# V-Sense/LFBM5D

Hardware: AMD Instinct MI355X
Metric: SAI-megapixels/sec (HT+Wiener, sigma=25) (higher is better)
Workload: dtype f32; 1 GPU; lf17x17x512x512_sigma25; light_field=17x17x512x512x3, asw=1, color_space=opp, noise=MT19937 seed 1 (utilities.cpp:176-183), window_lanes=2, spatial_bands=1, parallelism=single GPU

## Files before the change

### lfbm5d_amd/core.py

```python
import ctypes as C
import os
import subprocess

from typing import NamedTuple, Optional

import numpy as np

_HERE = os.path.dirname(os.path.abspath(__file__))

YUV, YCBCR, OPP, RGB, ID, DCT, SADCT, BIOR, HADAMARD, HAAR = range(10)
ROWMAJOR, COLMAJOR = 11, 12
TAU = {"id": ID, "dct": DCT, "sadct": SADCT, "bior": BIOR, "hw": HADAMARD, "haar": HAAR}
COLOR_SPACE = {"yuv": YUV, "ycbcr": YCBCR, "opp": OPP, "rgb": RGB}
UNIQUE_ID_BYTES = 128
SR_BICUBIC, SR_GAUSSIAN = 0, 1
SR_UP, SR_DOWN = 0, 1
SR_KERNEL = {"bicubic": SR_BICUBIC, "gaussian": SR_GAUSSIAN}


class LfBm5dError(RuntimeError):
    pass


class Params(C.Structure):
# ... 274 lines not shown
    out = (C.c_void_p * len(arrays))()
    for i, a in enumerate(arrays):
        if a is None or not mask[i]:
            continue
        if not (isinstance(a, np.ndarray) and a.dtype == np.float32 and a.flags.c_contiguous):
            raise LfBm5dError("per-SAI host buffers must be contiguous float32 numpy arrays")
        out[i] = a.ctypes.data
    return out


OPTION_ENV = ("LFBM5D_LANES", "LFBM5D_EMULATE_WORLD", "LFBM5D_MAX_WINDOWS", "LFBM5D_FUSED", "LFBM5D_STEP_SHARDING",
              "LFBM5D_DATA_DRIVEN_SCHEDULE", "LFBM5D_HOST_BLOCKING", "LFBM5D_BAND_MB", "LFBM5D_BM3D_LANES", "LFBM5D_SCAN_LDS_CAP",
              "LFBM5D_FORCE_REDO", "LFBM5D_SPATIAL_BANDS", "LFBM5D_BAND_HALO", "LFBM5D_SCAN_V1", "LFBM5D_SCAN_ANY", "LFBM5D_SCAN_FULL_TABLES", "LFBM5D_DCT8W_V2",
              "LFBM5D_GROUP_GENERIC", "LFBM5D_NO_SA_KERNELS", "LFBM5D_NO_SLAB_KERNEL", "LFBM5D_WIDE_NOSPLIT", "LFBM5D_AGG_64BIT",
              "LFBM5D_AGG_SCALAR_SCAN", "LFBM5D_SUBSET_LIST_HOST", "LFBM5D_SUBSET_SCAN_V1", "LFBM5D_FILT_GROUP_MAJOR",
              "LFBM5D_HT_REF_ORDER", "LFBM5D_WINDOW_SUMS_PADDED")
OPTION_ENV_EMPTY_OFF = ("LFBM5D_WINDOW_SUMS_PADDED",)


class Context:

    def __init__(self, device=0):
        self._L = lib()
        h = C.c_void_p()
        if self._L.lfbm5d_create(C.byref(h), int(device)) != 0:
            raise LfBm5dError(self._L.lfbm5d_last_error(None).decode())
        self._handle = h
        self._env_seen = {k: os.environ.get(k) for k in OPTION_ENV}
        self.device = int(device)

    @property
# ... 330 lines not shown
```

### lfbm5d_amd/csrc/lfbm5d_aggregate.hip

```cpp
#include "lfbm5d_kernels.h"

#include <algorithm>
#include <cstdlib>

namespace lfbm5d {

namespace {



constexpr int kAggFlush = 64;
template <bool WINDOWED, int TW, int TH, int kAggPF, int kAggU, bool BIG, bool VEC4>
__global__ __launch_bounds__(64) __attribute__((amdgpu_waves_per_eu((VEC4 && TW == 8 && !BIG) ? 8 : 1))) void k_aggregate(AggArgs a) {
    constexpr int kAggCap = kAggFlush + kAggPF * 64 + kAggU;
    __shared__ uint4 hit_a[kAggCap];
    __shared__ float hit_w2[kAggCap];
    __shared__ float kai[WINDOWED ? 256 : 1];
    const int lane = threadIdx.x;
    const unsigned org = a.direct ? a.nHW : 0u, Wt = a.Wb - 2 * org, Ht = a.Hb - 2 * org;
    const unsigned gx = (Wt + TW - 1) / TW, gy = (Ht + TH - 1) / TH, total_wg = gx * gy * a.A;
    const unsigned per_xcd = gridDim.x / 8;
    const unsigned lin2 = (blockIdx.x % 8) * per_xcd + blockIdx.x / 8;
    if (lin2 >= total_wg) return;
    const int st = (int)(lin2 / (gx * gy));
    const int tile_y = (int)((lin2 / gx) % gy), tile_x = (int)(lin2 % gx);
    if (a.proc_bits.test((unsigned)st)) return;
    if (!a.mask_bits.test((unsigned)st)) return;
    const int tx0 = (int)org + tile_x * TW, ty0 = (int)org + tile_y * TH;
    const int x = tx0 + lane % TW, y = ty0 + lane / TW;
    const bool inside = x < (int)(org + Wt) && y < (int)(org + Ht);
    const int k = a.k, k2 = k * k, C = a.C, N = a.N, A = a.A;
// ... 26 lines not shown
    const size_t pix = (a.direct ? (size_t)a.sai.st[st] * a.lf_stride : (size_t)st * C * plane) + (size_t)(y - (int)org) * Wt + (size_t)(x - (int)org);
    if (inside) for (int c = 0; c < C; c++) { accn[c] = a.num[pix + c * plane]; accd[c] = a.den[pix + c * plane]; }

    const bool mul_div = !a.irregular && (long long)n_rr * ncols_span < (1 << 20);
    const unsigned div_m = ((1u << 20) + (unsigned)max(ncols_span, 1) - 1) / (unsigned)max(ncols_span, 1);
    const unsigned g_end = a.ref_begin + a.n_groups;
    const bool sai_major = a.filt_sai_stride != 0;
    const unsigned Af = sai_major ? 1u : (unsigned)A, stf = sai_major ? 0u : (unsigned)st;
    const float* const filt = a.filt + (sai_major ? (size_t)st * a.filt_sai_stride : (size_t)0);
    const unsigned long long filt_bytes = sai_major ? a.filt_sai_stride * sizeof(float) : a.filt_bytes;
    const bool small24 = (((unsigned long long)a.n_refs_total << logN) + 1) * Af < (1ull << 24);
    const unsigned* apos = a.aggpos + (size_t)st * a.n_refs_total * N;
    const unsigned cstride = C > 1 ? (unsigned)k2 * 4u : 0u;
    const __amdgpu_buffer_rsrc_t rs_filt = __builtin_amdgcn_make_buffer_rsrc((void*)filt, 0, BIG ? 0 : (int)(unsigned)filt_bytes, 0x00020000u);
    unsigned nh = 0;

    auto consume = [&]() {
        const unsigned nh_pad = (nh + kAggU - 1) / kAggU * kAggU;
        if (nh + lane < nh_pad) { hit_a[nh + lane] = make_uint4(0xffffffffu, 0u, 0u, 0u); hit_w2[nh + lane] = 0.0f; }
        __builtin_amdgcn_wave_barrier();
        for (unsigned h0 = 0; h0 < nh_pad; h0 += kAggU) {
            float val[kAggU][3], kw[kAggU][3];
#pragma unroll
            for (int u = 0; u < kAggU; u++) {
                const uint4 ha = hit_a[h0 + u];
                const float w2 = hit_w2[h0 + u];
                const int dy = y - (int)(ha.x >> 16), dx = x - (int)(ha.x & 0xffffu);
                const bool on = (unsigned)dy < (unsigned)k && (unsigned)dx < (unsigned)k;
                const unsigned o = __umul24((unsigned)min(max(dy, 0), k - 1), (unsigned)k) + (unsigned)min(max(dx, 0), k - 1);
                const float kz = WINDOWED ? kai[o] : 1.0f;
                if (BIG) {
                    const char* fp = reinterpret_cast<const char*>(filt) + ((size_t)ha.y + o) * 4;
                    val[u][0] = *reinterpret_cast<const float*>(fp);
                    val[u][1] = *reinterpret_cast<const float*>(fp + cstride);
                    val[u][2] = *reinterpret_cast<const float*>(fp + 2 * cstride);
                } else {
                    const int vo = (int)((ha.y + o) * 4u);
                    val[u][0] = __builtin_bit_cast(float, __builtin_amdgcn_raw_buffer_load_b32(rs_filt, vo, 0, kFiltLoadAux));
                    val[u][1] = __builtin_bit_cast(float, __builtin_amdgcn_raw_buffer_load_b32(rs_filt, vo, (int)cstride, kFiltLoadAux));
                    val[u][2] = __builtin_bit_cast(float, __builtin_amdgcn_raw_buffer_load_b32(rs_filt, vo, (int)(2 * cstride), kFiltLoadAux));
                }
                kw[u][0] = on ? kz * __uint_as_float(ha.z) : 0.0f;
                kw[u][1] = on ? kz * __uint_as_float(ha.w) : 0.0f;
                kw[u][2] = on ? kz * w2 : 0.0f;
            }
// ... 43 lines not shown
            auto below = [&](unsigned long long b) { return __builtin_amdgcn_mbcnt_hi((unsigned)(b >> 32), __builtin_amdgcn_mbcnt_lo((unsigned)b, 0u)); };
            const unsigned total = (unsigned)__popcll(b0) + 2u * (unsigned)__popcll(b1) + 4u * (unsigned)__popcll(b2);
            if (nh + total > cap_hits) return false;
            if (m4) {
                unsigned slot = nh + below(b0) + 2u * below(b1) + 4u * below(b2);
                size_t wbase; unsigned off;
                const unsigned gl = g - a.ref_begin;
                if (small24) { wbase = __umul24(g, (unsigned)C); off = __umul24(__umul24((gl << logN) + n0, Af) + stf, (unsigned)(C * k2)); }
                else { asm volatile("" ::: "memory"); wbase = (size_t)g * C; off = (((gl << logN) + n0) * Af + stf) * C * k2; }
                float w[3];
#pragma unroll
                for (int c = 0; c < 3; c++) w[c] = c < C ? a.wgt[wbase + (a.wchan0 ? 0 : c)] : 0.0f;
#pragma unroll
                for (int j = 0; j < 4; j++) {
                    if (m4 & (1u << j)) {
                        hit_a[slot] = make_uint4(pj[j], off, __float_as_uint(w[0]), __float_as_uint(w[1]));
                        hit_w2[slot] = w[2];
                        slot++;
                    }
                    off += pstep;
                }
            }
            nh += total;
            __builtin_amdgcn_wave_barrier();
            return true;
        };
        for (int c0 = 0; c0 < n_cand; c0 += 256) {
            if (!try_append(c0, 0u, 64u))
                for (unsigned l0 = 0; l0 < 64; l0 += 16) { consume(); (void)try_append(c0, l0, l0 + 16); }
            if (nh >= kAggFlush) consume();
        }
    } else
// ... 30 lines not shown
        for (int u = 0; u < kAggPF; u++) {
            const int py = (int)(p[u] >> 16), px = (int)(p[u] & 0xffffu);
            hit[u] = p[u] != 0xffffffffu && py < ty0 + TH && py + k > ty0 && px < tx0 + TW && px + k > tx0;
#pragma unroll
            for (int c = 0; c < 3; c++) w[u][c] = (hit[u] && c < C) ? a.wgt[wbase[u] + (a.wchan0 ? 0 : c)] : 0.0f;
        }
#pragma unroll
        for (int u = 0; u < kAggPF; u++) {
            const unsigned long long bal = __ballot(hit[u]);
            if (hit[u]) {
                const unsigned slot = nh + __popcll(bal & ((1ull << lane) - 1ull));
                unsigned off;
                const unsigned gl = g[u] - a.ref_begin;
                if (small24) off = __umul24(__umul24((gl << logN) + nn[u], Af) + stf, (unsigned)(C * k2));
                else { asm volatile("" ::: "memory"); off = (((gl << logN) + nn[u]) * Af + stf) * C * k2; }
                hit_a[slot] = make_uint4(p[u], off, __float_as_uint(w[u][0]), __float_as_uint(w[u][1]));
                hit_w2[slot] = w[u][2];
            }
            nh += __popcll(bal);
        }
        __builtin_amdgcn_wave_barrier();
        if (nh >= kAggFlush) consume();
    }
    if (nh) consume();
    if (inside) for (int c = 0; c < C; c++) { a.num[pix + c * plane] = accn[c]; a.den[pix + c * plane] = accd[c]; }
}

}

hipError_t launch_aggregate(hipStream_t s, const AggArgs& a) {
    const bool wide = a.k >= 12;
    constexpr int kAgg16TW = 16, kAgg16TH = 4, kAgg8TW = 8, kAgg8TH = 8;
    const unsigned tw = wide ? (a.k == 12 ? 16 : kAgg16TW) : (a.k == 8 ? kAgg8TW : 8), th = wide ? (a.k == 12 ? 4 : kAgg16TH) : (a.k == 8 ? kAgg8TH : 8);
    const unsigned org = a.direct ? a.nHW : 0u;
    const unsigned tiles = ((a.Wb - 2 * org + tw - 1) / tw) * ((a.Hb - 2 * org + th - 1) / th) * a.A;
    const dim3 grid(((tiles + 7) / 8) * 8), block(64);
    const bool big = (a.filt_sai_stride ? a.filt_sai_stride * sizeof(float) : a.filt_bytes) > 0xfffff000ull || (a.opt & kOptAgg64Bit);
    const bool vec4 = a.N % 4 == 0 && !wide && !(a.opt & kOptAggScalarScan);
#define LFBM5D_AGG(W_, TW_, TH_, PF_, U_) \
    do { if (big && vec4) hipLaunchKernelGGL((k_aggregate<W_, TW_, TH_, PF_, U_, true, true>), grid, block, 0, s, a); \
         else if (big)    hipLaunchKernelGGL((k_aggregate<W_, TW_, TH_, PF_, U_, true, false>), grid, block, 0, s, a); \
         else if (vec4)   hipLaunchKernelGGL((k_aggregate<W_, TW_, TH_, PF_, U_, false, true>), grid, block, 0, s, a); \
         else             hipLaunchKernelGGL((k_aggregate<W_, TW_, TH_, PF_, U_, false, false>), grid, block, 0, s, a); } while (0)
    constexpr int kAgg16PF = 3, kAgg16U = 12, kAgg8PF = 3, kAgg8U = 6;
    if (a.k == 12)      LFBM5D_AGG(true, 16, 4, 3, 12);
    else if (a.k == 8)  LFBM5D_AGG(true, kAgg8TW, kAgg8TH, kAgg8PF, kAgg8U);
    else if (wide)      LFBM5D_AGG(false, kAgg16TW, kAgg16TH, kAgg16PF, kAgg16U);
    else                LFBM5D_AGG(false, 8, 8, 2, 6);
#undef LFBM5D_AGG
    return hipGetLastError();
}

}
```

### lfbm5d_amd/csrc/lfbm5d_group_generic.hip

```cpp
#include "lfbm5d_group_device.h"

namespace lfbm5d {

namespace {

__global__ __launch_bounds__(256) void k_group_pos(GroupArgs a) {
    const int A = a.A, N = a.N, NA = N * A;
    const size_t plane = (size_t)a.Wb * a.Hb;
    const size_t idx = (size_t)blockIdx.x * blockDim.x + threadIdx.x;
    if (idx == 0 && a.sa_list) a.sa_list[0] = 0u;
    if (idx >= (size_t)a.n_groups * N) return;
    const unsigned g = a.ref_begin + (unsigned)(idx / N);
    const int n = (int)(idx % N);
    const int nSx = (int)a.self_cnt[g];
    const unsigned k_r = a.refs[g];
    const unsigned ind_pst = n < nSx ? a.self_idx[(size_t)g * N + n] : 0u;
    const bool want_ofs = A == 9 && a.tau2 == 4 && a.step == 1 && (size_t)A * a.C * plane * 4 < 0x7fffffffull;
    unsigned bits = 0;
    for (int st = 0; st < A; st++) {
        const bool masked = a.mask_bits.test((unsigned)st);
        unsigned p = 0xffffffffu;
        if (n < nSx && masked) p = (st == (int)a.pst) ? ind_pst : a.best[(size_t)st * plane + ind_pst];
        const bool zero_patch = a.fill_quirk && p != 0xffffffffu && (p % a.Wb) >= a.Wb - a.k;
        const int i = n * A + st;
        a.gpos[(size_t)g * NA + i] = zero_patch ? 0xffffffffu : p;
        if (want_ofs) {
            const bool there = !zero_patch && p != 0xffffffffu;
            a.gofs[(size_t)g * NA + i] = there ? (unsigned)(((size_t)st * a.C * plane + p) * 4) : 0u;
            bits |= there ? 1u << st : 0u;
        }
        const bool in_shape = st == (int)a.pst || (masked && a.shape[(size_t)st * plane + k_r]);
        a.aggpos[((size_t)st * a.n_refs_total + g) * N + n] = ((a.tau4 != 6 || in_shape) && p != 0xffffffffu) ? ((p / a.Wb) << 16) | (p % a.Wb) : 0xffffffffu;
    }
    if (want_ofs) a.gok[(size_t)g * N + n] = bits;
}
template <bool BIG>
__global__ __launch_bounds__(256) void k_group_shape(GroupArgs a) {
    typedef typename std::conditional<BIG, ShapeInfoBig, ShapeInfo>::type SH;
    const unsigned i = blockIdx.x * blockDim.x + threadIdx.x;
    if (i >= a.n_groups) return;
    const unsigned g = a.ref_begin + i;
    const size_t plane = (size_t)a.Wb * a.Hb;
    const unsigned k_r = a.refs[g];
    SH* out = reinterpret_cast<SH*>(a.gshape) + g;
    if (a.tau4 != 6) { out->use_sadct = 0; return; }
    const int A = (int)a.A, aw = window_side(A);
    if (BIG) {
        int* m = out->mask_dct;
        int full = 0;
// ... 318 lines not shown
```

### lfbm5d_amd/csrc/lfbm5d_group_ht.hip

```cpp
#include "lfbm5d_group_device.h"

namespace lfbm5d {

namespace {

__device__ __forceinline__ constexpr float ht_guard(int st) { return st == 0 ? 1.0f / 65536.0f : (st == 3 || st == 6) ? 1.0f / 131072.0f : 1.0f / 262144.0f; }
template <int NS> __device__ __forceinline__ void haar_fwd_pairs_u(v2f* P) {
    if (NS == 8) {
        const v2f S01 = P[0] + P[1], D01 = P[0] - P[1], S23 = P[2] + P[3], D23 = P[2] - P[3];
        const v2f SS = S01 + S23, DD = S01 - S23;
        P[0] = v2f{SS.x + SS.y, SS.x - SS.y}; P[1] = DD; P[2] = D01; P[3] = D23;
    } else if (NS == 4) {
        const v2f S = P[0] + P[1], D = P[0] - P[1];
        P[0] = v2f{S.x + S.y, S.x - S.y}; P[1] = D;
    } else if (NS == 2) {
        P[0] = v2f{P[0].x + P[0].y, P[0].x - P[0].y};
    }
}
template <int NS> __device__ __forceinline__ void haar_inv_pairs_u(v2f* P) {
    if (NS == 8) {
        const v2f X = v2f{P[0].x + P[0].y, P[0].x - P[0].y};
        const v2f U = P[1] * 2.0f + X, V = X - P[1] * 2.0f, D01 = P[2], D23 = P[3];
        P[0] = D01 * 4.0f + U; P[1] = U - D01 * 4.0f; P[2] = D23 * 4.0f + V; P[3] = V - D23 * 4.0f;
    } else if (NS == 4) {
// ... 163 lines not shown
}

template <int NS, bool HAAR, bool LDSW = false, int SA_MODE = 0, bool FAST = false>
__device__ __forceinline__ bool group_id_body(const GroupArgs& a, unsigned g, int c, int pq, const __attribute__((address_space(4))) unsigned* pos,
                                              ShRef sh, bool use_sadct, float& wacc, float& s1, float& s2, float* work = nullptr) {
    const int k = a.k, k2 = k * k, A = 9;
    const unsigned plane = a.Wb * a.Hb;
    const unsigned kRsrcFlags = 0x00020000u;
    const __amdgpu_buffer_rsrc_t rs_in = __builtin_amdgcn_make_buffer_rsrc((void*)a.noisy, 0, (int)((size_t)a.A * a.C * plane * 4), kRsrcFlags);
    float* const out = a.filt + (size_t)g * a.N * A * a.C * k2;
    const __amdgpu_buffer_rsrc_t rs_out = __builtin_amdgcn_make_buffer_rsrc((void*)out, 0, (int)((size_t)a.N * A * a.C * k2 * 4), kRsrcFlags);
    constexpr int NH = NS > 1 ? NS / 2 : 1;
    v2f V[NH][9];
    const int voff = (int)(((unsigned)(pq / k) * a.Wb + pq % k) * 4u);
    const int woff = (pq / k) * (k + 1) + pq % k;
    unsigned okbits[NS];
    typedef const __attribute__((address_space(4))) unsigned* cuptr_;
    const cuptr_ ofs = (cuptr_)(a.gofs + (size_t)g * a.N * A), ok = (cuptr_)(a.gok + (size_t)g * a.N);
    const unsigned cbase = (unsigned)c * plane * 4u;
    auto load_all = [&]() {
        if (LDSW) {
#pragma unroll
            for (int n = 0; n < NS; n++)
#pragma unroll
                for (int st = 0; st < 9; st++) {
                    const float x = work[(n * A + st) * kT16Patch + woff];
                    if (n < NH) V[n][st].x = x; else V[n - NH][st].y = x;
                    okbits[n] = 0x1ffu;
                }
        } else
#pragma unroll
        for (int n = 0; n < NS; n++) {
            okbits[n] = ok[n];
#pragma unroll
            for (int st = 0; st < 9; st++) {
                const unsigned so = ofs[n * A + st] + cbase;
                const float x = __builtin_bit_cast(float, __builtin_amdgcn_raw_buffer_load_b32(rs_in, voff, (int)so, 0));
                if (n < NH) V[n][st].x = x; else V[n - NH][st].y = x;
            }
        }
        if (NS == 1) {
#pragma unroll
            for (int st = 0; st < 9; st++) V[0][st].y = 0.0f;
        }
#pragma unroll
        for (int n = 0; n < NS; n++)
            if (okbits[n] != 0x1ffu) {
#pragma unroll
                for (int st = 0; st < 9; st++) {
                    if (n < NH) V[n][st].x = ((okbits[n] >> st) & 1) ? V[n][st].x : 0.0f;
                    else V[n - NH][st].y = ((okbits[n] >> st) & 1) ? V[n - NH][st].y : 0.0f;
                }
            }
    };
    load_all();
    bool near = false;
    if (FAST) near = group_id_compute_fast<NS>(a, c, V, wacc, s1, s2);
    else
    group_id_compute<NS, HAAR, SA_MODE>(a, c, sh, use_sadct, V, wacc, s1, s2);
    const int vout = pq * 4;
#pragma unroll
    for (int n = 0; n < NS; n++)
#pragma unroll
        for (int st = 0; st < 9; st++) {
            const float r = n < NH ? V[n][st].x : V[n - NH][st].y;
            if (LDSW) work[(n * A + st) * kT16Patch + woff] = r;
            else __builtin_amdgcn_raw_buffer_store_b32(__builtin_bit_cast(int, r), rs_out, vout, (int)((((unsigned)(n * A + st) * a.C + c) * k2) * 4u), kFiltStoreAux);
        }
    return near;
}

template <bool HAAR, int SA_MODE, bool FAST = false>
__device__ __forceinline__ void group_id_one(const GroupArgs& a, const unsigned g, const int c, float (*red)[4]) {
    const int tid = threadIdx.x;
    const int A = 9, N = a.N;
    const int nSx = (int)a.self_cnt[g];
    typedef const __attribute__((address_space(4))) unsigned* cuptr;
    const cuptr pos = (cuptr)(a.gpos + (size_t)g * N * A);
    ShRef sh = group_shape(a, g);
    const bool use_sadct = a.tau4 == 6 && sh.use_sadct;
    if (SA_MODE == 3 && use_sadct) return;
    float wacc = 0.0f, s1 = 0.0f, s2 = 0.0f;
// ... 311 lines not shown
}

hipError_t prepare_group_ht() {
    const void* fns[] = {
        reinterpret_cast<const void*>(&k_group_bior16_haar), reinterpret_cast<const void*>(&k_group_bior16_any),
        reinterpret_cast<const void*>(&k_group_dct16_haar), reinterpret_cast<const void*>(&k_group_dct16_any),
        reinterpret_cast<const void*>(&k_group_bior16_n1), reinterpret_cast<const void*>(&k_group_dct16_n1),
        reinterpret_cast<const void*>(&k_group_bior16_n1_sa), reinterpret_cast<const void*>(&k_group_dct16_n1_sa)};
    for (const void* f : fns) {
        const hipError_t e = hipFuncSetAttribute(f, hipFuncAttributeMaxDynamicSharedMemorySize, kDedicatedLdsLimit);
        if (e != hipSuccess) return e;
    }
    return hipSuccess;
}

hipError_t launch_group_ht(hipStream_t s, const GroupArgs& a, bool all_sa, bool* launched) {
    *launched = true;
    if (a.tau2 == 4 && a.N <= 8 && a.k * a.k <= 256 && a.step == 1 && a.A == 9 && (size_t)a.A * a.C * a.Wb * a.Hb * 4 < 0x7fffffffull) {
        const unsigned threads = ((a.k * a.k + 63) / 64) * 64;
        const unsigned gx = ((a.n_groups + 7) / 8) * 8;
        if (all_sa) {
            if (a.tau5 == 9) hipLaunchKernelGGL(k_group_id_haar_sa, dim3(gx, a.C), dim3(threads), 0, s, a);
            else             hipLaunchKernelGGL(k_group_id_any_sa, dim3(gx, a.C), dim3(threads), 0, s, a);
        }
        else {
            if (!a.sa_list) return hipErrorInvalidValue;
            const bool fast = a.tau5 == 9 && (a.tau4 == 5 || a.tau4 == 6) && a.C <= 3 && !(a.opt & kOptHtReferenceOrder);
            if (fast)             hipLaunchKernelGGL(k_group_id_haar_fast, dim3(gx, a.C), dim3(threads), 0, s, a);
            else if (a.tau5 == 9) hipLaunchKernelGGL(k_group_id_haar, dim3(gx, a.C), dim3(threads), 0, s, a);
            else                  hipLaunchKernelGGL(k_group_id_any, dim3(gx, a.C), dim3(threads), 0, s, a);
            if (a.tau4 == 6 || fast) {
                if (a.tau5 == 9) hipLaunchKernelGGL(k_group_id_haar_list, dim3(kSaListBlocks), dim3(threads), 0, s, a);
                else             hipLaunchKernelGGL(k_group_id_any_list, dim3(kSaListBlocks), dim3(threads), 0, s, a);
// ... 32 lines not shown
```

### lfbm5d_amd/csrc/lfbm5d_kernels.h

```cpp
#ifndef LFBM5D_KERNELS_H
#define LFBM5D_KERNELS_H

#include <hip/hip_runtime.h>
#include <vector>

#include "lfbm5d_options.h"

constexpr int kFiltStoreAux = 2;
constexpr int kFiltLoadAux = 0;

#if defined(__HIPCC__)
typedef float filt_v4f __attribute__((ext_vector_type(4)));
typedef float filt_v2f __attribute__((ext_vector_type(2)));
__device__ __forceinline__ void filt_put(float* p, const float v) { *p = v; }
__device__ __forceinline__ void filt_put2(filt_v2f* p, const filt_v2f v) { *p = v; }
__device__ __forceinline__ void filt_put4(filt_v4f* p, const filt_v4f v) { *p = v; }
__device__ __forceinline__ void filt_put4(float4* p, const float4 v) { *p = v; }
__device__ __forceinline__ void filt_put4_nt(filt_v4f* p, const filt_v4f v) { __builtin_nontemporal_store(v, p); }
#endif

namespace lfbm5d {

constexpr int kMaxK = 32;
constexpr int kMaxA = 49;
// ... 69 lines not shown
    unsigned ref_begin, n_groups;
    unsigned Wb, Hb, C, A, k, N, pst;
    SaiMask mask_bits, proc_bits;
    unsigned tau2, tau4, tau5, useSD;
    unsigned fill_quirk;
    int step;
    float lambda;
    float sigma[3];
    float ht3_T[3][9][4];
    float ht3_K[3][9];
    float* scratch;
    unsigned long long scratch_floats;
    unsigned opt;
    unsigned long long filt_sai_stride;
    unsigned bm3d;
};

constexpr unsigned kSaiMajorMinA = 121;
__device__ __forceinline__ size_t filt_patch(const GroupArgs& a, unsigned g, unsigned n, unsigned st, unsigned k2) {
    return a.filt_sai_stride ? (size_t)st * a.filt_sai_stride + ((size_t)g * a.N + n) * a.C * k2
                             : (((size_t)g * a.N + n) * a.A + st) * a.C * k2;
}


struct SaiList { unsigned st[kBigA]; unsigned n; };

struct AggArgs {
    float* num;
    float* den;
    const float* filt;
// ... 6 lines not shown
    const unsigned* self_idx;
    const unsigned* self_cnt;
    const unsigned* best;
    const unsigned char* shape;
    const GroupTables* tb;
    unsigned ref_begin, n_groups;
    unsigned n_ref_rows, n_ref_cols;
    unsigned Wb, Hb, C, A, k, N, pst, p, nHW, nSim, nDisp;
    SaiMask mask_bits, proc_bits; unsigned tau4;
    unsigned irregular;
    unsigned opt;
    unsigned wchan0;
    unsigned direct;
    unsigned long long lf_stride;
    SaiList sai;
};

__host__ __device__ inline size_t stereo_table_stride(unsigned W, unsigned H, unsigned k, unsigned nDisp) {
    const unsigned ncols = W - 2 * nDisp - (k - 1), nrows = H - 2 * nDisp - (k - 1);
    return (size_t)((ncols + 63) / 64) * 64 * (nrows + 63);
}

__host__ __device__ inline unsigned stereo_table_srq(unsigned H, unsigned k, unsigned nDisp) {
    const unsigned nrows = H - 2 * nDisp - (k - 1);
    return ((nrows - 1 + 63 + 15) / 16) * 4 + 1;
}
__host__ __device__ inline size_t stereo_table_stride2(unsigned W, unsigned H, unsigned k, unsigned nDisp) {
    const unsigned ncols = W - 2 * nDisp - (k - 1);
    return (size_t)((ncols - 1 + 63) / 64) * stereo_table_srq(H, k, nDisp) * 256 + stereo_table_srq(H, k, nDisp) * 4;
}
// ... 106 lines not shown
                                 unsigned* best, unsigned char* shape);
hipError_t launch_stereo_argmin2(hipStream_t s, const float* tables, const unsigned* st_of_slot, unsigned n_slots,
                                 unsigned W, unsigned H, unsigned k, unsigned nDisp, float thr,
                                 unsigned* best, unsigned char* shape);
hipError_t launch_self_select(hipStream_t s, const float* scores, const unsigned* refs, unsigned n_refs,
                              unsigned W, unsigned nSim, unsigned N, float thr, unsigned* self_idx,
                              unsigned* self_cnt,
                              unsigned grid_cols = 0, unsigned nHW = 0, unsigned p = 1, unsigned last_r = 0, unsigned last_c = 0);
hipError_t launch_self_trivial(hipStream_t s, const unsigned* refs, unsigned n_refs, unsigned* self_idx,
                               unsigned* self_cnt);
hipError_t launch_stereo_argmin(hipStream_t s, const float* tables, const unsigned* st_of_slot, unsigned n_slots,
                                unsigned W, unsigned H, unsigned k, unsigned nDisp, float thr,
                                unsigned* best, unsigned char* shape);
hipError_t prepare_group_kernels();
hipError_t launch_group(hipStream_t s, const GroupArgs& a);
size_t group_lds_bytes(const GroupArgs& a);
size_t group_scratch_bytes(const GroupArgs& a);
hipError_t launch_aggregate(hipStream_t s, const AggArgs& a);

}
#endif
```

### lfbm5d_amd/csrc/lfbm5d_options.h

```cpp
#ifndef LFBM5D_OPTIONS_H
#define LFBM5D_OPTIONS_H

#include <cstddef>
#include <cstdlib>
#include <cstring>
#include <string>

namespace lfbm5d {

enum : unsigned {
    kOptScanV1 = 1u << 0,
    kOptScanAny = 1u << 1,
    kOptScanFullTables = 1u << 2,
    kOptDct8wV2 = 1u << 3,
    kOptGroupGeneric = 1u << 4,
    kOptNoSaKernels = 1u << 5,
    kOptNoSlabKernel = 1u << 6,
    kOptWideNoSplit = 1u << 7,
    kOptAgg64Bit = 1u << 8,
    kOptAggScalarScan = 1u << 9,
    kOptSubsetListHost = 1u << 10,
    kOptSubsetScanV1 = 1u << 11,
    kOptFiltGroupMajor = 1u << 12,
    kOptHtReferenceOrder = 1u << 13,
};

struct Options {
    int lanes = 2;
    int emulate_world = 0;
    int max_windows = 0;
    int fused = 1;
    int step_sharding = 0;
    int data_driven_schedule = 0;
    int host_blocking = 0;
    int band_mb = 0;
    int bm3d_lanes = 3;
    int scan_lds_cap = 0;
    int force_redo = 0;
    int spatial_bands = 1;
// ... 11 lines not shown
        {"step_sharding", "LFBM5D_STEP_SHARDING", &Options::step_sharding, 0},
        {"data_driven_schedule", "LFBM5D_DATA_DRIVEN_SCHEDULE", &Options::data_driven_schedule, 0},
        {"host_blocking", "LFBM5D_HOST_BLOCKING", &Options::host_blocking, 0}, {"band_mb", "LFBM5D_BAND_MB", &Options::band_mb, 0},
        {"bm3d_lanes", "LFBM5D_BM3D_LANES", &Options::bm3d_lanes, 0}, {"scan_lds_cap", "LFBM5D_SCAN_LDS_CAP", &Options::scan_lds_cap, 0},
        {"force_redo", "LFBM5D_FORCE_REDO", &Options::force_redo, 0}, {"spatial_bands", "LFBM5D_SPATIAL_BANDS", &Options::spatial_bands, 0},
        {"band_halo", "LFBM5D_BAND_HALO", &Options::band_halo, 0},
        {"window_sums_padded", "LFBM5D_WINDOW_SUMS_PADDED", &Options::window_sums_padded, 0},
        {"scan_v1", "LFBM5D_SCAN_V1", nullptr, kOptScanV1}, {"scan_any", "LFBM5D_SCAN_ANY", nullptr, kOptScanAny},
        {"scan_full_tables", "LFBM5D_SCAN_FULL_TABLES", nullptr, kOptScanFullTables}, {"dct8w_v2", "LFBM5D_DCT8W_V2", nullptr, kOptDct8wV2},
        {"group_generic", "LFBM5D_GROUP_GENERIC", nullptr, kOptGroupGeneric}, {"no_sa_kernels", "LFBM5D_NO_SA_KERNELS", nullptr, kOptNoSaKernels},
        {"no_slab_kernel", "LFBM5D_NO_SLAB_KERNEL", nullptr, kOptNoSlabKernel}, {"wide_nosplit", "LFBM5D_WIDE_NOSPLIT", nullptr, kOptWideNoSplit},
        {"agg_64bit", "LFBM5D_AGG_64BIT", nullptr, kOptAgg64Bit}, {"agg_scalar_scan", "LFBM5D_AGG_SCALAR_SCAN", nullptr, kOptAggScalarScan},
        {"subset_list_host", "LFBM5D_SUBSET_LIST_HOST", nullptr, kOptSubsetListHost}, {"subset_scan_v1", "LFBM5D_SUBSET_SCAN_V1", nullptr, kOptSubsetScanV1},
        {"filt_group_major", "LFBM5D_FILT_GROUP_MAJOR", nullptr, kOptFiltGroupMajor},
        {"ht_reference_order", "LFBM5D_HT_REF_ORDER", nullptr, kOptHtReferenceOrder},
    };
    *n = sizeof(keys) / sizeof(keys[0]);
    return keys;
}

inline bool option_set(Options& o, const char* key, const char* value) {
    size_t n; const OptionKey* keys = option_keys(&n);
    static const Options defaults;
    for (size_t i = 0; i < n; i++) {
        if (std::strcmp(key, keys[i].key) != 0 && std::strcmp(key, keys[i].env) != 0) continue;
        const bool unset = value == nullptr || value[0] == 0;
        if (keys[i].field) {
            int v = defaults.*(keys[i].field);
            if (!unset) {
                if (keys[i].field == &Options::step_sharding) v = std::strcmp(value, "rows") == 0 ? 1 : std::strcmp(value, "blocks") == 0 ? 2 : std::atoi(value);
// ... 36 lines not shown
```

### lfbm5d_amd/csrc/lfbm5d_pass.hip

```cpp
#include "lfbm5d_ctx.h"

namespace lfbm5d_host {

lfbm5d_ctx* new_ctx(int device, std::string& err) {
    hipError_t e;
    lfbm5d_ctx* c = new lfbm5d_ctx();
    c->device = device;
    std::memset(&c->stats, 0, sizeof(c->stats));
    if ((e = hipStreamCreateWithFlags(&c->stream, hipStreamNonBlocking)) != hipSuccess) { err = hipGetErrorString(e); delete c; return nullptr; }
    if ((e = prepare_group_kernels()) != hipSuccess || (e = prepare_scan2_kernels()) != hipSuccess) { err = std::string("kernel LDS limits: ") + hipGetErrorString(e); (void)hipStreamDestroy(c->stream); delete c; return nullptr; }
    if ((e = hipHostMalloc((void**)&c->h_small, 64 * sizeof(unsigned))) != hipSuccess) { err = hipGetErrorString(e); (void)hipStreamDestroy(c->stream); delete c; return nullptr; }
    return c;
}


hipEvent_t get_event(lfbm5d_ctx* c) {
    if (c->ev_used == c->ev_pool.size()) {
        hipEvent_t e; (void)hipEventCreate(&e); c->ev_pool.push_back(e);
    }
    return c->ev_pool[c->ev_used++];
}

void drain_events(lfbm5d_ctx* c) {
    for (const PassEvents& pe : c->pending) {
// ... 260 lines not shown
    {
        constexpr size_t kFiltCapBytes = (size_t)12 << 30;
        size_t cap = std::min<size_t>(kFiltCapBytes, (size_t)0xfff00000ull * sizeof(float));
        if (c->opt->band_mb > 0) cap = std::min<size_t>(cap, (size_t)c->opt->band_mb << 20);
        const size_t row_groups = centre ? gc.n_ref_cols : 1;
        if ((size_t)R * per_group * sizeof(float) > cap) {
            const size_t rows_fit = std::max<size_t>(1, cap / (per_group * sizeof(float) * row_groups));
            band_groups = (unsigned)std::min<size_t>(R, rows_fit * row_groups);
        }
    }
    HIPCK(c, c->filt.reserve((size_t)band_groups * per_group * sizeof(float)));
    HIPCK(c, c->wgt.reserve((size_t)R * C * sizeof(float)));
    HIPCK(c, c->aggpos.reserve((size_t)A * R * Nst * sizeof(unsigned)));
    HIPCK(c, c->gpos.reserve((size_t)A * R * Nst * sizeof(unsigned)));
    HIPCK(c, c->gofs.reserve((size_t)A * R * Nst * sizeof(unsigned)));
    HIPCK(c, c->gok.reserve((size_t)R * Nst * sizeof(unsigned)));
    HIPCK(c, c->sa_list.reserve((size_t)(4 * (size_t)R + 1) * sizeof(unsigned)));
    HIPCK(c, c->gshape.reserve((size_t)R * (A > (unsigned)kMaxA ? kShapeInfoBigBytes : kShapeInfoBytes)));
    HIPCK(c, gc.tb.reserve(sizeof(GroupTables)));
    if (!c->counters.p) {
        HIPCK(c, c->counters.reserve(32 * sizeof(unsigned long long)));
        HIPCK(c, hipMemsetAsync(c->counters.p, 0, 32 * sizeof(unsigned long long), s));
    }
    unsigned long long* const d_counters = c->counters.as<unsigned long long>() + 16 * c->gslot;
    if (gc.tb_key[0] != k || gc.tb_key[1] != aw || gc.tb_key[2] != ah) {
        GroupTables tb;
        build_tables(tb, k, aw, ah);
        HIPCK(c, hipMemcpyAsync(gc.tb.p, &tb, sizeof(tb), hipMemcpyHostToDevice, s));
        HIPCK(c, hipStreamSynchronize(s));
        gc.tb_key[0] = k; gc.tb_key[1] = aw; gc.tb_key[2] = ah;
    }
// ... 109 lines not shown
    ga.opt = c->opt->kernels;
    if (const size_t sb = group_scratch_bytes(ga)) {
        HIPCK(c, c->gscratch.reserve(sb));
        ga.scratch = c->gscratch.as<float>(); ga.scratch_floats = sb / sizeof(float);
    }
    AggArgs aa;
    std::memset(&aa, 0, sizeof(aa));
    aa.num = d_num; aa.den = d_den; aa.wgt = ga.wgt; aa.aggpos = ga.aggpos; aa.n_refs_total = R; aa.refs = ga.refs;
    aa.self_idx = ga.self_idx; aa.self_cnt = ga.self_cnt; aa.best = ga.best; aa.shape = ga.shape; aa.tb = ga.tb;
    aa.ref_begin = ref_begin; aa.n_groups = n_groups; aa.n_ref_rows = gc.n_ref_rows; aa.n_ref_cols = gc.n_ref_cols;
    aa.Wb = Wb; aa.Hb = Hb; aa.C = C; aa.A = A; aa.k = k; aa.N = Nst; aa.pst = pst; aa.p = P->p;
    aa.nHW = nHW; aa.nSim = P->nSim; aa.nDisp = P->nDisp;
    aa.mask_bits = mask_bits; aa.proc_bits = proc_bits; aa.tau4 = P->tau_4D; aa.irregular = centre ? 0u : 1u;
    aa.wchan0 = (bm3d && P->useSD) ? 1u : 0u;
    aa.opt = c->opt->kernels;
    if (direct) {
        aa.num = c->direct.num; aa.den = c->direct.den; aa.direct = 1u; aa.lf_stride = c->direct.lf_stride; aa.sai = c->direct.sai;
    }
    const bool sai_major = A >= kSaiMajorMinA && !(c->opt->kernels & kOptFiltGroupMajor);
    const size_t per_group_bias = sai_major ? per_group / A : per_group;
    if (n_groups <= band_groups) {
        ga.filt_sai_stride = aa.filt_sai_stride = sai_major ? (unsigned long long)n_groups * (per_group / A) : 0ull;
        ga.filt = c->filt.as<float>() - (size_t)ref_begin * per_group_bias;
        aa.filt = c->filt.as<float>(); aa.filt_bytes = (unsigned long long)n_groups * per_group * sizeof(float);
        if (n_groups) HIPCK(c, launch_group(s, ga));
        HIPCK(c, hipEventRecord(pe.e[2], s));
        if (n_groups) HIPCK(c, launch_aggregate(s, aa));
        HIPCK(c, hipEventRecord(pe.e[3], s));
    } else {
        bool first = true;
// ... 57 lines not shown
```

Baseline: 252.9 SAI-megapixels/s.

## Store filtered HT patches in tile-split row-block layout for aggregation locality

Adds a split layout for filtered group patches when k=16. The HT group kernel writes each patch split at the aggregation tile boundary into left and right pieces. Within each piece, rows are blocked in groups of 4, so an aggregation tile reads its columns from contiguous memory. The group kernel stores a per-SAI split column in an extra gok word, and the aggregate kernel gets a BR template instance that recomputes offsets from the piece width. This trades more offset arithmetic, extra LDS and a doubled gok buffer for better-coalesced filter loads in aggregation. It is on by default and can be turned off with LFBM5D_FILT_ROWS.

Measured after the change: 250.2 SAI-megapixels/s. -1.0%, worse.

```diff
diff --git a/lfbm5d_amd/core.py b/lfbm5d_amd/core.py
--- a/lfbm5d_amd/core.py
+++ b/lfbm5d_amd/core.py
@@ -312,7 +312,7 @@
               "LFBM5D_FORCE_REDO", "LFBM5D_SPATIAL_BANDS", "LFBM5D_BAND_HALO", "LFBM5D_SCAN_V1", "LFBM5D_SCAN_ANY", "LFBM5D_SCAN_FULL_TABLES", "LFBM5D_DCT8W_V2",
               "LFBM5D_GROUP_GENERIC", "LFBM5D_NO_SA_KERNELS", "LFBM5D_NO_SLAB_KERNEL", "LFBM5D_WIDE_NOSPLIT", "LFBM5D_AGG_64BIT",
               "LFBM5D_AGG_SCALAR_SCAN", "LFBM5D_SUBSET_LIST_HOST", "LFBM5D_SUBSET_SCAN_V1", "LFBM5D_FILT_GROUP_MAJOR",
-              "LFBM5D_HT_REF_ORDER", "LFBM5D_WINDOW_SUMS_PADDED")
+              "LFBM5D_HT_REF_ORDER", "LFBM5D_WINDOW_SUMS_PADDED", "LFBM5D_FILT_ROWS")
 OPTION_ENV_EMPTY_OFF = ("LFBM5D_WINDOW_SUMS_PADDED",)
 
 
diff --git a/lfbm5d_amd/csrc/lfbm5d_aggregate.hip b/lfbm5d_amd/csrc/lfbm5d_aggregate.hip
--- a/lfbm5d_amd/csrc/lfbm5d_aggregate.hip
+++ b/lfbm5d_amd/csrc/lfbm5d_aggregate.hip
@@ -10,11 +10,12 @@
 
 
 constexpr int kAggFlush = 64;
-template <bool WINDOWED, int TW, int TH, int kAggPF, int kAggU, bool BIG, bool VEC4>
+template <bool WINDOWED, int TW, int TH, int kAggPF, int kAggU, bool BIG, bool VEC4, int BR>
 __global__ __launch_bounds__(64) __attribute__((amdgpu_waves_per_eu((VEC4 && TW == 8 && !BIG) ? 8 : 1))) void k_aggregate(AggArgs a) {
     constexpr int kAggCap = kAggFlush + kAggPF * 64 + kAggU;
     __shared__ uint4 hit_a[kAggCap];
     __shared__ float hit_w2[kAggCap];
+    __shared__ unsigned short hit_pw[BR ? kAggCap : 1];
     __shared__ float kai[WINDOWED ? 256 : 1];
     const int lane = threadIdx.x;
     const unsigned org = a.direct ? a.nHW : 0u, Wt = a.Wb - 2 * org, Ht = a.Hb - 2 * org;
@@ -71,10 +72,19 @@
     const unsigned cstride = C > 1 ? (unsigned)k2 * 4u : 0u;
     const __amdgpu_buffer_rsrc_t rs_filt = __builtin_amdgcn_make_buffer_rsrc((void*)filt, 0, BIG ? 0 : (int)(unsigned)filt_bytes, 0x00020000u);
     unsigned nh = 0;
+    auto piece_bias = [&](const unsigned pos) -> unsigned {
+        if (!BR) return 0u;
+        const int px = (int)(pos & 0xffffu);
+        return filt_piece_bias(TW, BR, filt_split_s(TW, px, (int)org), px >= tx0);
+    };
+    auto piece_w = [&](const unsigned pos) -> unsigned {
+        const int px = (int)(pos & 0xffffu);
+        return filt_piece_w(TW, filt_split_s(TW, px, (int)org), px >= tx0);
+    };
 
     auto consume = [&]() {
         const unsigned nh_pad = (nh + kAggU - 1) / kAggU * kAggU;
-        if (nh + lane < nh_pad) { hit_a[nh + lane] = make_uint4(0xffffffffu, 0u, 0u, 0u); hit_w2[nh + lane] = 0.0f; }
+        if (nh + lane < nh_pad) { hit_a[nh + lane] = make_uint4(0xffffffffu, 0u, 0u, 0u); hit_w2[nh + lane] = 0.0f; if (BR) hit_pw[nh + lane] = (unsigned short)TW; }
         __builtin_amdgcn_wave_barrier();
         for (unsigned h0 = 0; h0 < nh_pad; h0 += kAggU) {
             float val[kAggU][3], kw[kAggU][3];
@@ -84,8 +94,9 @@
                 const float w2 = hit_w2[h0 + u];
                 const int dy = y - (int)(ha.x >> 16), dx = x - (int)(ha.x & 0xffffu);
                 const bool on = (unsigned)dy < (unsigned)k && (unsigned)dx < (unsigned)k;
-                const unsigned o = __umul24((unsigned)min(max(dy, 0), k - 1), (unsigned)k) + (unsigned)min(max(dx, 0), k - 1);
-                const float kz = WINDOWED ? kai[o] : 1.0f;
+                const unsigned orow = __umul24((unsigned)min(max(dy, 0), k - 1), (unsigned)k) + (unsigned)min(max(dx, 0), k - 1);
+                const float kz = WINDOWED ? kai[orow] : 1.0f;
+                const unsigned o = BR ? filt_piece_offset(TW, BR, (unsigned)hit_pw[BR ? h0 + u : 0], min(max(dy, 0), TW - 1), min(max(dx, 0), TW - 1)) : orow;
                 if (BIG) {
                     const char* fp = reinterpret_cast<const char*>(filt) + ((size_t)ha.y + o) * 4;
                     val[u][0] = *reinterpret_cast<const float*>(fp);
@@ -159,8 +170,9 @@
 #pragma unroll
                 for (int j = 0; j < 4; j++) {
                     if (m4 & (1u << j)) {
-                        hit_a[slot] = make_uint4(pj[j], off, __float_as_uint(w[0]), __float_as_uint(w[1]));
+                        hit_a[slot] = make_uint4(pj[j], off + piece_bias(pj[j]), __float_as_uint(w[0]), __float_as_uint(w[1]));
                         hit_w2[slot] = w[2];
+                        if (BR) hit_pw[slot] = (unsigned short)piece_w(pj[j]);
                         slot++;
                     }
                     off += pstep;
@@ -221,8 +233,9 @@
                 const unsigned gl = g[u] - a.ref_begin;
                 if (small24) off = __umul24(__umul24((gl << logN) + nn[u], Af) + stf, (unsigned)(C * k2));
                 else { asm volatile("" ::: "memory"); off = (((gl << logN) + nn[u]) * Af + stf) * C * k2; }
-                hit_a[slot] = make_uint4(p[u], off, __float_as_uint(w[u][0]), __float_as_uint(w[u][1]));
+                hit_a[slot] = make_uint4(p[u], off + piece_bias(p[u]), __float_as_uint(w[u][0]), __float_as_uint(w[u][1]));
                 hit_w2[slot] = w[u][2];
+                if (BR) hit_pw[slot] = (unsigned short)piece_w(p[u]);
             }
             nh += __popcll(bal);
         }
@@ -237,23 +250,26 @@
 
 hipError_t launch_aggregate(hipStream_t s, const AggArgs& a) {
     const bool wide = a.k >= 12;
-    constexpr int kAgg16TW = 16, kAgg16TH = 4, kAgg8TW = 8, kAgg8TH = 8;
-    const unsigned tw = wide ? (a.k == 12 ? 16 : kAgg16TW) : (a.k == 8 ? kAgg8TW : 8), th = wide ? (a.k == 12 ? 4 : kAgg16TH) : (a.k == 8 ? kAgg8TH : 8);
+    constexpr int kAgg16TW = agg_tile(16).tw, kAgg16TH = agg_tile(16).th, kAgg16BR = agg_tile(16).br, kAgg8TW = agg_tile(8).tw, kAgg8TH = agg_tile(8).th;
+    static_assert(agg_tile(12).tw == 16 && agg_tile(12).th == 4 && agg_tile(6).tw == 8 && agg_tile(6).th == 8 && kAgg16BR > 0 && kAgg16TW == 16, "instances below");
+    const unsigned tw = (unsigned)agg_tile(a.k).tw, th = (unsigned)agg_tile(a.k).th;
+    if (a.filt_split && !(a.k == 16 && agg_tile(a.k).br)) return hipErrorInvalidValue;
     const unsigned org = a.direct ? a.nHW : 0u;
     const unsigned tiles = ((a.Wb - 2 * org + tw - 1) / tw) * ((a.Hb - 2 * org + th - 1) / th) * a.A;
     const dim3 grid(((tiles + 7) / 8) * 8), block(64);
     const bool big = (a.filt_sai_stride ? a.filt_sai_stride * sizeof(float) : a.filt_bytes) > 0xfffff000ull || (a.opt & kOptAgg64Bit);
     const bool vec4 = a.N % 4 == 0 && !wide && !(a.opt & kOptAggScalarScan);
-#define LFBM5D_AGG(W_, TW_, TH_, PF_, U_) \
-    do { if (big && vec4) hipLaunchKernelGGL((k_aggregate<W_, TW_, TH_, PF_, U_, true, true>), grid, block, 0, s, a); \
-         else if (big)    hipLaunchKernelGGL((k_aggregate<W_, TW_, TH_, PF_, U_, true, false>), grid, block, 0, s, a); \
-         else if (vec4)   hipLaunchKernelGGL((k_aggregate<W_, TW_, TH_, PF_, U_, false, true>), grid, block, 0, s, a); \
-         else             hipLaunchKernelGGL((k_aggregate<W_, TW_, TH_, PF_, U_, false, false>), grid, block, 0, s, a); } while (0)
+#define LFBM5D_AGG(W_, TW_, TH_, PF_, U_, BR_) \
+    do { if (big && vec4) hipLaunchKernelGGL((k_aggregate<W_, TW_, TH_, PF_, U_, true, true, BR_>), grid, block, 0, s, a); \
+         else if (big)    hipLaunchKernelGGL((k_aggregate<W_, TW_, TH_, PF_, U_, true, false, BR_>), grid, block, 0, s, a); \
+         else if (vec4)   hipLaunchKernelGGL((k_aggregate<W_, TW_, TH_, PF_, U_, false, true, BR_>), grid, block, 0, s, a); \
+         else             hipLaunchKernelGGL((k_aggregate<W_, TW_, TH_, PF_, U_, false, false, BR_>), grid, block, 0, s, a); } while (0)
     constexpr int kAgg16PF = 3, kAgg16U = 12, kAgg8PF = 3, kAgg8U = 6;
-    if (a.k == 12)      LFBM5D_AGG(true, 16, 4, 3, 12);
-    else if (a.k == 8)  LFBM5D_AGG(true, kAgg8TW, kAgg8TH, kAgg8PF, kAgg8U);
-    else if (wide)      LFBM5D_AGG(false, kAgg16TW, kAgg16TH, kAgg16PF, kAgg16U);
-    else                LFBM5D_AGG(false, 8, 8, 2, 6);
+    if (a.k == 12)      LFBM5D_AGG(true, 16, 4, 3, 12, 0);
+    else if (a.k == 8)  LFBM5D_AGG(true, kAgg8TW, kAgg8TH, kAgg8PF, kAgg8U, 0);
+    else if (a.filt_split) LFBM5D_AGG(false, kAgg16TW, kAgg16TH, kAgg16PF, kAgg16U, kAgg16BR);
+    else if (wide)      LFBM5D_AGG(false, kAgg16TW, kAgg16TH, kAgg16PF, kAgg16U, 0);
+    else                LFBM5D_AGG(false, 8, 8, 2, 6, 0);
 #undef LFBM5D_AGG
     return hipGetLastError();
 }
diff --git a/lfbm5d_amd/csrc/lfbm5d_filt_layout.h b/lfbm5d_amd/csrc/lfbm5d_filt_layout.h
--- /dev/null
+++ b/lfbm5d_amd/csrc/lfbm5d_filt_layout.h
@@ -0,0 +1,43 @@
+#ifndef LFBM5D_FILT_LAYOUT_H
+#define LFBM5D_FILT_LAYOUT_H
+
+#if defined(__HIPCC__)
+#define LFBM5D_HD __host__ __device__
+#else
+#define LFBM5D_HD
+#endif
+
+namespace lfbm5d {
+
+struct AggTile { int tw, th, br; };
+LFBM5D_HD constexpr AggTile agg_tile(unsigned k) {
+    return k == 16 ? AggTile{16, 4, 4} : k >= 12 ? AggTile{16, 4, 0} : AggTile{8, 8, 0};
+}
+
+LFBM5D_HD constexpr int filt_split_s(int tw, int px, int org) {
+    const int m = (px - org) % tw;
+    return tw - (m < 0 ? m + tw : m);
+}
+
+struct FiltSplitPixel { unsigned ml, al, mr, ar; };
+LFBM5D_HD constexpr FiltSplitPixel filt_split_pixel(int k, int br, int y, int x) {
+    const int yy = y % br, blk = (y / br) * br * k;
+    return FiltSplitPixel{(unsigned)yy, (unsigned)(blk + x), (unsigned)(br - 1 - yy), (unsigned)(blk + yy * k + x)};
+}
+LFBM5D_HD constexpr unsigned filt_split_offset(int k, int br, int s, int y, int x) {
+    const FiltSplitPixel p = filt_split_pixel(k, br, y, x);
+    const unsigned sc = (unsigned)(s < k ? s : k);
+    return (unsigned)x < sc ? p.ml * sc + p.al : p.mr * sc + p.ar;
+}
+LFBM5D_HD constexpr unsigned filt_split_offset(int k, int tw, int br, int px, int org, int y, int x) {
+    return filt_split_offset(k, br, filt_split_s(tw, px, org), y, x);
+}
+
+LFBM5D_HD constexpr unsigned filt_piece_w(int k, int s, bool left) { return (unsigned)(left ? (s < k ? s : k) : k - (s < k ? s : k)); }
+LFBM5D_HD constexpr unsigned filt_piece_bias(int k, int br, int s, bool left) { return left ? 0u : (unsigned)((br - 1) * (s < k ? s : k)); }
+LFBM5D_HD constexpr unsigned filt_piece_offset(int k, int br, unsigned w, int y, int x) {
+    return (unsigned)((y / br) * br * k) + (unsigned)(y % br) * w + (unsigned)x;
+}
+
+}
+#endif
diff --git a/lfbm5d_amd/csrc/lfbm5d_group_generic.hip b/lfbm5d_amd/csrc/lfbm5d_group_generic.hip
--- a/lfbm5d_amd/csrc/lfbm5d_group_generic.hip
+++ b/lfbm5d_amd/csrc/lfbm5d_group_generic.hip
@@ -16,7 +16,8 @@
     const unsigned k_r = a.refs[g];
     const unsigned ind_pst = n < nSx ? a.self_idx[(size_t)g * N + n] : 0u;
     const bool want_ofs = A == 9 && a.tau2 == 4 && a.step == 1 && (size_t)A * a.C * plane * 4 < 0x7fffffffull;
-    unsigned bits = 0;
+    unsigned bits = 0, split_lo = 0;
+    const int tw = agg_tile(a.k).tw;
     for (int st = 0; st < A; st++) {
         const bool masked = a.mask_bits.test((unsigned)st);
         unsigned p = 0xffffffffu;
@@ -28,11 +29,15 @@
             const bool there = !zero_patch && p != 0xffffffffu;
             a.gofs[(size_t)g * NA + i] = there ? (unsigned)(((size_t)st * a.C * plane + p) * 4) : 0u;
             bits |= there ? 1u << st : 0u;
+            if (a.filt_split) {
+                const unsigned s1 = min((unsigned)filt_split_s(tw, p != 0xffffffffu ? (int)(p % a.Wb) : 0, (int)a.agg_org), a.k) - 1u;
+                if (st < 8) split_lo |= s1 << (4 * st); else bits |= s1 << 16;
+            }
         }
         const bool in_shape = st == (int)a.pst || (masked && a.shape[(size_t)st * plane + k_r]);
         a.aggpos[((size_t)st * a.n_refs_total + g) * N + n] = ((a.tau4 != 6 || in_shape) && p != 0xffffffffu) ? ((p / a.Wb) << 16) | (p % a.Wb) : 0xffffffffu;
     }
-    if (want_ofs) a.gok[(size_t)g * N + n] = bits;
+    if (want_ofs) { a.gok[((size_t)g * N + n) * 2] = bits; a.gok[((size_t)g * N + n) * 2 + 1] = split_lo; }
 }
 template <bool BIG>
 __global__ __launch_bounds__(256) void k_group_shape(GroupArgs a) {
diff --git a/lfbm5d_amd/csrc/lfbm5d_group_ht.hip b/lfbm5d_amd/csrc/lfbm5d_group_ht.hip
--- a/lfbm5d_amd/csrc/lfbm5d_group_ht.hip
+++ b/lfbm5d_amd/csrc/lfbm5d_group_ht.hip
@@ -201,9 +201,9 @@
     v2f V[NH][9];
     const int voff = (int)(((unsigned)(pq / k) * a.Wb + pq % k) * 4u);
     const int woff = (pq / k) * (k + 1) + pq % k;
-    unsigned okbits[NS];
+    unsigned okbits[NS], splits[NS];
     typedef const __attribute__((address_space(4))) unsigned* cuptr_;
-    const cuptr_ ofs = (cuptr_)(a.gofs + (size_t)g * a.N * A), ok = (cuptr_)(a.gok + (size_t)g * a.N);
+    const cuptr_ ofs = (cuptr_)(a.gofs + (size_t)g * a.N * A), ok = (cuptr_)(a.gok + (size_t)g * a.N * 2);
     const unsigned cbase = (unsigned)c * plane * 4u;
     auto load_all = [&]() {
         if (LDSW) {
@@ -213,12 +213,12 @@
                 for (int st = 0; st < 9; st++) {
                     const float x = work[(n * A + st) * kT16Patch + woff];
                     if (n < NH) V[n][st].x = x; else V[n - NH][st].y = x;
-                    okbits[n] = 0x1ffu;
+                    okbits[n] = 0x1ffu; splits[n] = 0u;
                 }
         } else
 #pragma unroll
         for (int n = 0; n < NS; n++) {
-            okbits[n] = ok[n];
+            okbits[n] = ok[2 * n]; splits[n] = ok[2 * n + 1];
 #pragma unroll
             for (int st = 0; st < 9; st++) {
                 const unsigned so = ofs[n * A + st] + cbase;
@@ -232,7 +232,7 @@
         }
 #pragma unroll
         for (int n = 0; n < NS; n++)
-            if (okbits[n] != 0x1ffu) {
+            if ((okbits[n] & 0x1ffu) != 0x1ffu) {
 #pragma unroll
                 for (int st = 0; st < 9; st++) {
                     if (n < NH) V[n][st].x = ((okbits[n] >> st) & 1) ? V[n][st].x : 0.0f;
@@ -245,14 +245,23 @@
     if (FAST) near = group_id_compute_fast<NS>(a, c, V, wacc, s1, s2);
     else
     group_id_compute<NS, HAAR, SA_MODE>(a, c, sh, use_sadct, V, wacc, s1, s2);
-    const int vout = pq * 4;
+    FiltSplitPixel fp = FiltSplitPixel{0u, (unsigned)pq, 0u, (unsigned)pq};
+    if (!LDSW && a.filt_split) fp = k == 16 ? filt_split_pixel(16, agg_tile(16).br, pq >> 4, pq & 15) : filt_split_pixel(k, max(agg_tile(a.k).br, 1), pq / k, pq % k);
+    const unsigned px_in = k == 16 ? (unsigned)(pq & 15) : (unsigned)(pq % k);
+    unsigned ml4 = fp.ml * 4u, al4 = (fp.al + fp.ml) * 4u, mr4 = fp.mr * 4u, ar4 = (fp.ar + fp.mr) * 4u;
+    asm volatile("" : "+v"(ml4), "+v"(al4), "+v"(mr4), "+v"(ar4));
 #pragma unroll
     for (int n = 0; n < NS; n++)
 #pragma unroll
         for (int st = 0; st < 9; st++) {
             const float r = n < NH ? V[n][st].x : V[n - NH][st].y;
             if (LDSW) work[(n * A + st) * kT16Patch + woff] = r;
-            else __builtin_amdgcn_raw_buffer_store_b32(__builtin_bit_cast(int, r), rs_out, vout, (int)((((unsigned)(n * A + st) * a.C + c) * k2) * 4u), kFiltStoreAux);
+            else {
+                const unsigned s1 = st < 8 ? (splits[n] >> (4 * st)) & 15u : (okbits[n] >> 16) & 15u;
+                const bool left = px_in <= s1;
+                const int vo = (int)(__umul24(left ? ml4 : mr4, s1) + (left ? al4 : ar4));
+                __builtin_amdgcn_raw_buffer_store_b32(__builtin_bit_cast(int, r), rs_out, vo, (int)((((unsigned)(n * A + st) * a.C + c) * k2) * 4u), kFiltStoreAux);
+            }
         }
     return near;
 }
@@ -594,9 +603,14 @@
     return hipSuccess;
 }
 
+static bool ht_register_form(const GroupArgs& a) {
+    return a.tau2 == 4 && a.N <= 8 && a.k * a.k <= 256 && a.step == 1 && a.A == 9 && (size_t)a.A * a.C * a.Wb * a.Hb * 4 < 0x7fffffffull;
+}
+bool group_writes_split(const GroupArgs& a) { return ht_register_form(a) && !(a.opt & kOptGroupGeneric) && !a.bm3d && !a.filt_sai_stride; }
+
 hipError_t launch_group_ht(hipStream_t s, const GroupArgs& a, bool all_sa, bool* launched) {
     *launched = true;
-    if (a.tau2 == 4 && a.N <= 8 && a.k * a.k <= 256 && a.step == 1 && a.A == 9 && (size_t)a.A * a.C * a.Wb * a.Hb * 4 < 0x7fffffffull) {
+    if (ht_register_form(a)) {
         const unsigned threads = ((a.k * a.k + 63) / 64) * 64;
         const unsigned gx = ((a.n_groups + 7) / 8) * 8;
         if (all_sa) {
diff --git a/lfbm5d_amd/csrc/lfbm5d_kernels.h b/lfbm5d_amd/csrc/lfbm5d_kernels.h
--- a/lfbm5d_amd/csrc/lfbm5d_kernels.h
+++ b/lfbm5d_amd/csrc/lfbm5d_kernels.h
@@ -5,6 +5,7 @@
 #include <vector>
 
 #include "lfbm5d_options.h"
+#include "lfbm5d_filt_layout.h"
 
 constexpr int kFiltStoreAux = 2;
 constexpr int kFiltLoadAux = 0;
@@ -107,6 +108,7 @@
     unsigned opt;
     unsigned long long filt_sai_stride;
     unsigned bm3d;
+    unsigned filt_split, agg_org;
 };
 
 constexpr unsigned kSaiMajorMinA = 121;
@@ -143,6 +145,7 @@
     unsigned direct;
     unsigned long long lf_stride;
     SaiList sai;
+    unsigned filt_split;
 };
 
 __host__ __device__ inline size_t stereo_table_stride(unsigned W, unsigned H, unsigned k, unsigned nDisp) {
@@ -279,6 +282,7 @@
                                 unsigned* best, unsigned char* shape);
 hipError_t prepare_group_kernels();
 hipError_t launch_group(hipStream_t s, const GroupArgs& a);
+bool group_writes_split(const GroupArgs& a);
 size_t group_lds_bytes(const GroupArgs& a);
 size_t group_scratch_bytes(const GroupArgs& a);
 hipError_t launch_aggregate(hipStream_t s, const AggArgs& a);
diff --git a/lfbm5d_amd/csrc/lfbm5d_options.h b/lfbm5d_amd/csrc/lfbm5d_options.h
--- a/lfbm5d_amd/csrc/lfbm5d_options.h
+++ b/lfbm5d_amd/csrc/lfbm5d_options.h
@@ -23,6 +23,7 @@
     kOptSubsetScanV1 = 1u << 11,
     kOptFiltGroupMajor = 1u << 12,
     kOptHtReferenceOrder = 1u << 13,
+    kOptFiltRows = 1u << 14,
 };
 
 struct Options {
@@ -64,6 +65,7 @@
         {"subset_list_host", "LFBM5D_SUBSET_LIST_HOST", nullptr, kOptSubsetListHost}, {"subset_scan_v1", "LFBM5D_SUBSET_SCAN_V1", nullptr, kOptSubsetScanV1},
         {"filt_group_major", "LFBM5D_FILT_GROUP_MAJOR", nullptr, kOptFiltGroupMajor},
         {"ht_reference_order", "LFBM5D_HT_REF_ORDER", nullptr, kOptHtReferenceOrder},
+        {"filt_rows", "LFBM5D_FILT_ROWS", nullptr, kOptFiltRows},
     };
     *n = sizeof(keys) / sizeof(keys[0]);
     return keys;
diff --git a/lfbm5d_amd/csrc/lfbm5d_pass.hip b/lfbm5d_amd/csrc/lfbm5d_pass.hip
--- a/lfbm5d_amd/csrc/lfbm5d_pass.hip
+++ b/lfbm5d_amd/csrc/lfbm5d_pass.hip
@@ -298,7 +298,7 @@
     HIPCK(c, c->aggpos.reserve((size_t)A * R * Nst * sizeof(unsigned)));
     HIPCK(c, c->gpos.reserve((size_t)A * R * Nst * sizeof(unsigned)));
     HIPCK(c, c->gofs.reserve((size_t)A * R * Nst * sizeof(unsigned)));
-    HIPCK(c, c->gok.reserve((size_t)R * Nst * sizeof(unsigned)));
+    HIPCK(c, c->gok.reserve((size_t)R * Nst * 2 * sizeof(unsigned)));
     HIPCK(c, c->sa_list.reserve((size_t)(4 * (size_t)R + 1) * sizeof(unsigned)));
     HIPCK(c, c->gshape.reserve((size_t)R * (A > (unsigned)kMaxA ? kShapeInfoBigBytes : kShapeInfoBytes)));
     HIPCK(c, gc.tb.reserve(sizeof(GroupTables)));
@@ -438,6 +438,8 @@
     aa.mask_bits = mask_bits; aa.proc_bits = proc_bits; aa.tau4 = P->tau_4D; aa.irregular = centre ? 0u : 1u;
     aa.wchan0 = (bm3d && P->useSD) ? 1u : 0u;
     aa.opt = c->opt->kernels;
+    ga.agg_org = direct ? nHW : 0u;
+    ga.filt_split = aa.filt_split = (!(c->opt->kernels & kOptFiltRows) && group_writes_split(ga) && agg_tile(k).br > 0) ? 1u : 0u;
     if (direct) {
         aa.num = c->direct.num; aa.den = c->direct.den; aa.direct = 1u; aa.lf_stride = c->direct.lf_stride; aa.sai = c->direct.sai;
     }
```
